# jinseikenai/glomeruli_segmentation

Measured on AMD Instinct MI355X. Metric: patches/sec (1024x512 RGB) ESPNet p=2 q=8 5 classes, HBM-resident, two batches in flight, higher is better.
Workload: dtype f32; 1 GPU; ESPNet p=2 q=8 encoder+decoder, batch=32 synthetic 1024x512 uint8 BGR tiles per GPU, normalise+forward+argmax+counts, inputs resident in HBM, steps rotate through 4 distinct batches, 2 batch(es) in flight (engine lanes, one HIP stream each) for `value`; global_batch=32, weights=espnet_fold1 (tests/golden), parallelism=tile-range per rank x1

## Files before the change

### glomeruli_segmentation_amd/_lib.py

```python
import ctypes
import os

_PKG = os.path.dirname(os.path.abspath(__file__))
LIB_PATH = os.path.join(_PKG, "libglomseg.so")
if os.environ.get("GLOMSEG_LIB") and os.environ.get("GLOMSEG_EXPERIMENT") == "1":
    LIB_PATH = os.environ["GLOMSEG_LIB"]

GS_OK = 0
GS_IN_U8_BGR_NHWC = 0
GS_IN_F32_NCHW = 1
ABI_VERSION = 10
GS_BUILD_DIAG = 1
GS_FORM_NONE = -1
GS_MAX_ENSEMBLE_C = 8
MAX_CROPS_PER_CALL = 64

STATUS_NAMES = {0: "GS_OK", 1: "GS_ERR_INVALID", 2: "GS_ERR_HIP", 3: "GS_ERR_NOMEM", 4: "GS_ERR_UNSUPPORTED",
                5: "GS_ERR_NODEVICE", 6: "GS_ERR_DEVICE_FAULT"}


class GlomsegError(RuntimeError):
    def __init__(self, status, message):
        super().__init__("%s: %s" % (STATUS_NAMES.get(status, status), message))
        self.status = status
# ... 95 lines not shown
    "gs_arc_length_closed": (ctypes.c_double, [_P, _I]),
    "gs_approx_poly_closed": (_I, [_P, _I, ctypes.c_double, _P]),
    "gs_wsi_paste_max": (_I, [_P, _I, _I, _I, _P, _I, _I, _I, _I, _P]),
    "gs_wsi_paste_max_lut": (_I, [_P, _I, _I, _I, _P, _P, _P, _I, _I, _I, _I, _P]),
    "gs_overlay_classmap": (_I, [_P, _P, _I, _I, _P, _I, ctypes.c_float, ctypes.c_float, _P, _P]),
    "gs_confusion_u8": (_I, [_P, _P, ctypes.c_longlong, _I, _P, _P]),
    "gs_wsi_eval_windows": (_I, [_I, _I, _I, _I, ctypes.POINTER(EvalSet), ctypes.POINTER(EvalSet), _P, _P, _I, _I, _P, _P, _P]),
    "gs_conv2d_nhwc": (_I, [_P, _I, _I, _I, _I, _P, _I, _I, _I, _P, _I, _I, _I, _P, _P]),
    "gs_conv2d_nhwc_form": (_I, [_I] * 10 + [ctypes.POINTER(ctypes.c_char_p)]),
    "gs_roialign": (_I, [_P, _I, _I, _I, _I, _P, _P, _I, _I, _P, _P]),
    "gs_nms": (_I, [_P, _P, _I, ctypes.c_float, ctypes.c_float, _I, _P, _P, _P]),
    "gs_detector_create": (_I, [_P, ctypes.POINTER(LayerDesc), _I, ctypes.POINTER(_P)]),
    "gs_detector_destroy": (None, [_P]),
    "gs_detector_max_detections": (_I, []),
    "gs_detector_num_proposals": (_I, []),
    "gs_detector_layer_info": (_I, [_I, ctypes.POINTER(ctypes.c_char_p)] + [ctypes.POINTER(_I)] * 6),
    "gs_detector_plan": (_I, [_I, _I, _I, ctypes.POINTER(DetectorPlan)]),
    "gs_detector_set_thresholds": (_I, [_P, ctypes.c_float, ctypes.c_float, ctypes.c_float]),
    "gs_detector_forward": (_I, [_P, _P, _I, _I, _I, _P, _P, _P, _P, _P, _P, _P, _P, _P]),
    "gs_detector_detect_host": (_I, [_P, ctypes.POINTER(_P), _I, _I, _I, _I, _P, _P, _P, _P]),
}

SCORING_PROTOTYPES = {
    "gs_espnet_score_crops": (_I, [_P, _P, ctypes.POINTER(CropDesc), _I, _I, _I, _I, _P, _P, _P]),
    "gs_espnet_segment_crops_host_scored": (_I, PROTOTYPES["gs_espnet_segment_crops_host"][1] + [ctypes.POINTER(CropScoring)]),
}

PLAN_PROTOTYPES = {
    "gs_espnet_plan_flags": (_I, [_I, _I, _I, _I, _I, _I, _I, _I, ctypes.POINTER(_I)]),
    "gs_espnet_pack_weights": (_I, [_P, ctypes.POINTER(LayerDesc), _I, _I, _I, _I, _I, _P, ctypes.c_size_t, ctypes.POINTER(ctypes.c_size_t),
                                ctypes.POINTER(WeightPiece), _I, ctypes.POINTER(_I)]),
    "gs_espnet_workspace_plan": (_I, [_I] * 7 + [ctypes.POINTER(ctypes.c_size_t)]),
}
GS_PLAN_LAZY_B2, GS_PLAN_L3C_IN_REDUCE, GS_PLAN_CLS_IN_L3 = 1, 2, 4

INSTANCE_PROTOTYPES = {
    "gs_instances_plan": (_I, [_I, _I, _I, _I, ctypes.POINTER(ctypes.c_size_t)]),
    "gs_slide_instances": (_I, [_P, _I, _I, _I, _I, _P, ctypes.c_size_t, _I, _P, _P, _P, _P, _P]),
}

_lib = None


def load():
    global _lib
    if _lib is not None:
        return _lib
    if not os.path.exists(LIB_PATH):
        raise ImportError(
            "%s is missing: build it with `python -m glomeruli_segmentation_amd.build` "
            "(hipcc --offload-arch=gfx950).  There is no CPU fallback." % LIB_PATH)
    lib = ctypes.CDLL(LIB_PATH, mode=ctypes.RTLD_GLOBAL)
    for name, (res, args) in list(PROTOTYPES.items()) + list(SCORING_PROTOTYPES.items()) + list(PLAN_PROTOTYPES.items()) + \
            list(INSTANCE_PROTOTYPES.items()):
        if name in PLAN_PROTOTYPES and not hasattr(lib, name):
            continue
        fn = getattr(lib, name)
        fn.restype = res
        fn.argtypes = args
    if lib.gs_abi_version() != ABI_VERSION:
        raise ImportError("libglomseg.so ABI %d != binding ABI %d: rebuild" % (lib.gs_abi_version(), ABI_VERSION))
    if (lib.gs_build_flags() & GS_BUILD_DIAG) and os.environ.get("GLOMSEG_ALLOW_DIAG") != "1":
        raise ImportError("%s is a -DGS_DIAG experiment build (its timing variants return wrong results by construction); "
                          "set GLOMSEG_ALLOW_DIAG=1 to load it for an A/B measurement" % LIB_PATH)
    _lib = lib
    return lib

# ... 10 lines not shown
```

### glomeruli_segmentation_amd/build.py

```python
import os
import subprocess
import sys
import tempfile

PKG = os.path.dirname(os.path.abspath(__file__))
CSRC = os.path.join(PKG, "csrc")
LIB = os.path.join(PKG, "libglomseg.so")
SOURCES = ["espnet.hip", "dec_tail.hip", "crops.hip", "detect_ops.hip", "detector.hip", "wsi_eval.hip", "instances.hip", "contours.cpp"]
HEADERS = ["gs_internal.h", "conv_mfma.h", "dec_tail.h", "dec_tail_args.h", "espnet_kernels.h", "espnet_facts.h", "espnet_weights.h", "workspace_plan.h", "crop_sample.h", "crop_plan.h", "instance_plan.h", "detect_math.h", "detect_plan.h", "host_copy.h", "host_jobs.h", "host_pipe.h",
           os.path.join("..", "..", "include", "glomseg.h"), os.path.join("..", "..", "include", "glomseg_scoring.h"),
           os.path.join("..", "..", "include", "glomseg_plan.h"), os.path.join("..", "..", "include", "glomseg_instances.h")]
FLAGS = ["-O3", "--offload-arch=gfx950", "-std=c++17", "-fPIC", "-Wall", "-Wno-unused-result",
         "-Wno-unused-value"]


def _sources():
    return [s for s in SOURCES if os.path.exists(os.path.join(CSRC, s))]


def _stale(lib):
    if not os.path.exists(lib):
        return True
    t = os.path.getmtime(lib)
    deps = [os.path.join(CSRC, s) for s in _sources() + HEADERS] + [os.path.abspath(__file__)]
    deps += [os.path.join(CSRC, f) for f in os.listdir(CSRC) if f.endswith(".h") or f.endswith(".inc")]
    return any(os.path.getmtime(d) > t for d in deps)


def build_lib(force=False, verbose=False, out=None, extra_flags=()):
    lib = os.path.abspath(out) if out else LIB
    if not (force or _stale(lib)):
        return lib
    hipcc = os.environ.get("HIPCC", "/opt/rocm/bin/hipcc")
    os.makedirs(os.path.dirname(lib), exist_ok=True)
    objdir = CSRC if out is None else tempfile.mkdtemp(prefix="glomseg_obj_")
    objs = []
    procs = []
    for s in _sources():
        o = os.path.join(objdir, s.replace(".hip", ".o").replace(".cpp", ".o"))
        objs.append(o)
        cmd = [hipcc] + FLAGS + list(extra_flags) + (["-x", "hip"] if s.endswith(".cpp") else []) + ["-c", os.path.join(CSRC, s), "-o", o]
        if verbose:
# ... 21 lines not shown
```

### glomeruli_segmentation_amd/csrc/espnet.hip

```cpp
#include <chrono>
#include <cmath>
#include <cstdio>
#include <cstdlib>
#include <functional>
#include <map>
#include <memory>
#include <string>
#include <thread>
#include <vector>

#include "../../include/glomseg_plan.h"
#include "conv_mfma.h"
#include "dec_tail_args.h"
#include "enc_head.h"
#include "enc_head_ens.h"
#include "espnet_config.h"
#include "forward_plan.h"
#include "espnet_kernels.h"
#include "espnet_weights.h"
#include "host_copy.h"
#include "host_pipe.h"
#include "workspace_plan.h"

namespace gs {

static thread_local std::string g_err;
void set_error(const char *fmt, ...)
{
    char buf[1024];
    va_list ap;
    va_start(ap, fmt);
    vsnprintf(buf, sizeof buf, fmt, ap);
    va_end(ap);
    g_err = buf;
}

#ifdef GS_DIAG
static bool getenv_flag(const char *name)
{
    const char *e = std::getenv(name);
    return e && std::atoi(e) != 0;
}
static bool no_vec() { return getenv_flag("GS_NO_VEC"); }
#else
static constexpr bool no_vec() { return false; }
#endif

enum KernelId {
    K_STEM, K_POOL, K_L2_C1S, K_L2_DOWN, K_L2_C1, K_L2_ESP, K_CAT_B2, K_L3_C1S, K_L3_DOWN, K_L3_C1, K_L3_ESP,
    K_DEC1, K_DEC2, K_DEC3, K_DEC_CONV, K_DEC4, K_DEC_TAIL, K_ENC_HEAD, K_ENC_HEAD_ENS, K_COUNT
};
static const char *kKernelNames[K_COUNT] = {
    "stem_kernel", "pool_kernel", "conv_l2_reduce_s2", "conv_l2_down_branches", "conv_l2_reduce_1x1",
    "conv_l2_esp_branches", "cat_b2_kernel", "conv_l3_reduce_s2", "conv_l3_down_branches", "conv_l3_reduce_1x1",
    "conv_l3_esp_branches", "dec1_kernel", "dec2_kernel", "dec3_kernel", "conv_dec_cbr", "dec4_kernel", "dec_tail_kernel",
    "enc_head_kernel", "enc_head_ens_kernel"};

struct Model : Workspace {
    int classes = 0, p = 0, q = 0;
    int cp = 0;
    bool encoder_only = false;
    int device = 0, num_cus = 256;
#ifdef GS_DIAG
    int variant = 0;
#else
    static constexpr int variant = 0;
#endif
    float *dblob = nullptr;
    EspnetOffsets w;

    void *ws = nullptr;
    size_t ws_bytes = 0;
    int ws_n = 0, ws_h = 0, ws_w = 0;
    float *prob = nullptr;
    size_t prob_bytes = 0;
    std::map<std::string, std::pair<Act, int>> stages;
    void set_stage(const std::string &name, const Act &act, int C)
    {
        for (auto it = stages.begin(); it != stages.end();)
            it = it->second.first.base == act.base ? stages.erase(it) : std::next(it);
        stages[name] = {act, C};
    }
    int last_n = 0;
    bool b2_lazy = false;

    bool profile = false;
    struct Ev { hipEvent_t a, b; int k; };
    std::vector<Ev> events;
    double prof_ms[K_COUNT] = {0};
    long long prof_launches[K_COUNT] = {0};
    double prof_flops[K_COUNT] = {0};
};

static gs_status layout_workspace(Model *m, int n, int H, int W)
{
    if (m->ws && n <= m->ws_n && H == m->ws_h && W == m->ws_w)
        return GS_OK;
    if (m->ws) {
        GS_HIP(hipDeviceSynchronize());
        GS_HIP(hipFree(m->ws));
        m->ws = nullptr;
    }
    WorkspacePlan plan;
    const gs_status st = plan_workspace(n, H, W, m->cp, m->p, m->encoder_only, plan);
    if (st != GS_OK)
        return st;
    void *ws = nullptr;
    if (hipMalloc(&ws, plan.bytes) != hipSuccess) {
        set_error("workspace allocation of %zu bytes failed (n=%d, %dx%d)", plan.bytes, n, H, W);
        return GS_ERR_NOMEM;
    }
    GS_HIP(hipMemset(ws, 0, plan.bytes));
    GS_HIP(hipDeviceSynchronize());
    static_cast<Workspace &>(*m) = plan.acts;
    int i = 0;
    for (Act *a : acts_of(*m))
        a->base = reinterpret_cast<float *>(static_cast<char *>(ws) + plan.at[i++]);
// ... 396 lines not shown
            }
            ca = with_cls(ca, 0);
        }
        return launch_l3_down(m, plan.l3_down, plan.cls_in_l3, m->w.l3_0.fused_next ? with_fused(ca, m->r3[rd3 ^ 1], 25) : ca, s);
    });
    bool have_r3 = m->w.l3_0.fused_next;
    m->set_stage("level3_reduce", m->r3[rd3], 25);
    rd3 ^= have_r3 ? 1 : 0;
    m->set_stage("level3_0", m->cc[0], 128);
    int cur3 = 0;
    for (int i = 0; i < m->q; ++i) {
        const int nxt = cur3 == 1 ? 2 : 1;
        const bool fuse_next = m->w.l3[i].fused_next;
        if (!have_r3)
            L.run(K_L3_C1, px3 * (128 * 25 * 2), [&] {
                return launch_l3_c1(m, conv_args(m->cc[cur3], wb + m->w.l3[i].c1, m->r3[rd3], nullptr, n), s);
            });
        L.run(K_L3_ESP, px3 * (25 * 9 * 128 * 2) + (fuse_next ? px3 * (128 * 25 * 2) : 0) + (i == m->q - 1 ? cls_flops : 0), [&] {
            const ConvArgs ca = conv_args(m->r3[rd3], wb + m->w.l3[i].br, m->cc[nxt], &m->cc[cur3], n);
            GS_DIAG_TRY(diag_l3_esp(m, ca, i, s, dst_));
            if (fuse_next)
                return launch_l3_esp_fused(m, plan.l3_esp_fused, with_fused(ca, m->r3[rd3 ^ 1], 25), i, s);
            const bool cls5 = plan.cls_in_l3 && i == m->q - 1;
            return launch_l3_esp_last(m, plan.l3_esp_last, cls5, cls5 ? with_cls(ca, 1) : ca, s);
        });
        have_r3 = fuse_next;
        rd3 ^= have_r3 ? 1 : 0;
        cur3 = nxt;
        m->set_stage("level3." + std::to_string(i), m->cc[cur3], 128);
    }
    return {cur3, lazy_b2};
}

template <int CLS>
static gs_status decode(Model *m, Launcher &L, const ForwardPlan &plan, const ForwardReq &r, const Encoded &enc)
{
    const float *wb = m->dblob;
    const hipStream_t s = r.s;
    const int n = r.n, H = r.H, W = r.W, H1 = H / 2, W1 = W / 2, H2 = H / 4, W2 = W / 4, H3 = H / 8, W3 = W / 8;
    const double px1 = (double)H1 * W1, px2 = (double)H2 * W2, px3 = (double)H3 * W3;
    const int ncls = m->classes;
    float *enc_logits = !m->encoder_only ? nullptr : r.logits ? r.logits : m->o2c.base;
    L.run(K_DEC1, (plan.cls_in_l3 ? 0 : px3 * (256 * ncls * 2)) + px3 * (ncls * ncls * 4 * 2), [&] {
        if constexpr (CLS == CLS_N) {
            if (plan.cls_in_l3) {
                Dec1SumsArgs a{};
                a.part = m->tt.base;
                a.psn = m->tt.sn;
                a.psc = H3 * W3;
                a.br = wb + m->w.br;
                a.wup = wb + m->w.wup3;
                a.out = view(m->o2c);
                a.N = n;
                a.H3 = H3;
                a.W3 = W3;
                a.classes = ncls;
                hipLaunchKernelGGL(dec1_sums_kernel<CLS>, dim3(blocks_for((long long)n * H3 * W3)), dim3(256), 0, s, a);
                return GS_OK;
            }
        }
        Dec1Args a{};
        a.c0 = view(m->cc[0]);
        a.clast = view(m->cc[enc.last]);
        a.b3w = wb + m->w.b3;
        a.br = m->encoder_only ? nullptr : wb + m->w.br;
        a.wup = m->encoder_only ? nullptr : wb + m->w.wup3;
        a.out = view(m->o2c);
        a.enc_logits = enc_logits;
        a.N = n;
        a.classes = ncls;
        constexpr int CB = CLS <= 5 ? 16 : CLS <= 8 ? 8 : 4;
        hipLaunchKernelGGL((dec1_kernel<CLS, CB>), dim3((unsigned)(((long long)n * H3 * W3 + 63) / 64)), dim3(256), 0, s, a);
        return GS_OK;
    });
    if (m->encoder_only) {
        if (r.mask)
            L.run(K_ENC_HEAD, (double)H * W * (ncls * 6), [&] {
                EncHeadArgs a{};
                a.logits = enc_logits;
                a.mask = r.mask;
                a.hist = r.hist;
                a.classes = ncls;
                a.H3 = H3;
                a.W3 = W3;
                launch_enc_head(a, n, s);
                return GS_OK;
            });
        return L.st;
    }
    m->set_stage("up_l3", m->o2c, ncls);

    L.run(K_DEC2, plan.l3c_in_reduce ? 0 : px2 * (131 * ncls * 2), [&] {
        Dec2Args a{};
        a.o2c = view(m->o2c);
        a.br = wb + m->w.cbr0;
        a.t = view(m->tt);
        a.N = n;
        a.classes = ncls;
        if constexpr (l3c_side_sums(CLS)) {
            if (plan.l3c_in_reduce) {
                a.a1 = view(m->l3c);
                hipLaunchKernelGGL(dec2_br_kernel<CLS>, dim3(blocks_for((long long)n * H2 * W2)), dim3(256), 0, s, a);
                return GS_OK;
            }
        }
        a.a1 = view(m->a1);
        a.raw = view(m->bb[0]);
        a.b2 = wb + m->w.b2;
        a.raw_c0 = 64;
        a.raw_cn = enc.lazy_b2 ? 64 : 0;
        a.w3c = wb + m->w.w3c;
        hipLaunchKernelGGL(dec2_kernel<CLS>, dim3((unsigned)(((long long)n * H2 * W2 + 63) / 64)), dim3(256), 0, s, a);
        return GS_OK;
    });
    if (ncls == CLS)
        m->set_stage("combine_t", m->tt, 2 * CLS);
    if constexpr (dec3_on_mfma(CLS)) {
        L.run(K_DEC3, px2 * (2 * ncls * 9 * ncls * 2), [&] {
            return launch_dec3<CLS>(m, plan.dec3, conv_args(m->tt, wb + m->w.wcc_mfma, m->t3, nullptr, n), s);
        });
        L.run(K_DEC3, px2 * (ncls * ncls * 4 * 2), [&] {
            Dec3Args a{};
            a.t = view(m->t3);
            a.wup = wb + m->w.wup2;
            a.bnu = wb + m->w.bnu2;
            a.e = view(m->ee);
            a.N = n;
            a.classes = ncls;
            hipLaunchKernelGGL(dec3b_kernel<CLS>, dim3(blocks_for((long long)n * H2 * W2)), dim3(256), 0, s, a);
            return GS_OK;
        });
    } else {
        L.run(K_DEC3, px2 * (2 * ncls * 9 * ncls * 2) + px2 * (ncls * ncls * 4 * 2), [&] {
            Dec3Args a{};
            a.t = view(m->tt);
            a.wc = wb + m->w.wcc;
            a.bnc = wb + m->w.bncc;
            a.wup = wb + m->w.wup2;
            a.bnu = wb + m->w.bnu2;
            a.e = view(m->ee);
            a.N = n;
            a.classes = ncls;
            hipLaunchKernelGGL(dec3_kernel<CLS>, dim3(blocks_for((long long)n * H2 * W2)), dim3(256), 0, s, a);
            return GS_OK;
        });
    }
    m->set_stage("up_l2", m->ee, ncls);
    if constexpr (dec_tail_fused(CLS)) {
        L.run(K_DEC_TAIL, px1 * ((19 + CLS) * 9 * CLS * 2) + px1 * (CLS * CLS * 4 * 2), [&] {
            DecTailArgs a{};
            a.in = m->a0c.base;
            a.in_sn = m->a0c.sn;
            a.in_sc = m->a0c.sc;
            a.in_pitch = m->a0c.pitch;
            a.in_off = m->a0c.off;
            a.in_img_bytes = (unsigned)(m->a0c.sn * sizeof(float));
            a.wpack = wb + m->w.wtail;
            a.logits = r.logits;
            a.mask = r.mask;
            a.hist = ens_finishes((int)r.role) ? r.hist : nullptr;
            a.prob = r.prob;
            a.ens_mode = (int)r.role;
            a.ens_w = r.ens_w;
            if (r.logits) {
// ... 365 lines not shown
    GS_REQUIRE(h && in, "gs_espnet_forward: null handle or input");
    GS_REQUIRE(lane >= 0 && lane <= (int)h->lanes.size(), "lane %d does not exist (gs_espnet_set_lanes)", lane);
    gs_status st = check_shape(n, height, width);
    if (st != GS_OK) return st;
    GS_REQUIRE(in_format == GS_IN_U8_BGR_NHWC || in_format == GS_IN_F32_NCHW, "unknown input format %d", in_format);
    GS_REQUIRE(in_format != GS_IN_U8_BGR_NHWC || (mean && std), "uint8 input needs mean and std");
    GS_REQUIRE(logits || mask, "nothing to compute: logits and mask are both NULL");
    GS_REQUIRE(!hist || mask, "hist requires the mask output");
    if (in_format == GS_IN_U8_BGR_NHWC)
        for (int i = 0; i < 3; ++i)
            GS_REQUIRE(std[i] != 0.0f, "std[%d] is zero", i);
    ForwardReq r;
    r.in = in, r.in_format = in_format, r.n = n, r.H = height, r.W = width;
    r.mean = mean, r.stdv = std, r.logits = logits, r.mask = mask, r.hist = hist, r.s = static_cast<hipStream_t>(hip_stream);
    return espnet_forward(h, lane, r);
}

gs_status gs_espnet_read_stage(gs_espnet *h, const char *stage, int image, float *dst, size_t cap, int dims[3])
{
    GS_REQUIRE(h && stage && dims, "gs_espnet_read_stage: null argument");
    Model &m = h->m;
    auto it = m.stages.find(stage);
    GS_REQUIRE(it != m.stages.end(), "stage '%s' was not produced by the last forward", stage);
    GS_REQUIRE(image >= 0 && image < m.last_n, "image index %d out of range", image);
    const Act &a = it->second.first;
    const int C = it->second.second;
    dims[0] = C;
    dims[1] = a.H;
    dims[2] = a.W;
    const size_t count = (size_t)C * a.H * a.W;
    if (!dst)
        return GS_OK;
    GS_REQUIRE(cap >= count, "destination too small for stage '%s'", stage);
    float *tmp = nullptr;
    GS_HIP(hipMalloc(reinterpret_cast<void **>(&tmp), count * sizeof(float)));
    hipLaunchKernelGGL(unpad_kernel, dim3(blocks_for((long long)count)), dim3(256), 0, 0, view(a), image, C, tmp);
    if (m.b2_lazy && std::string(stage) == "b2")
        hipLaunchKernelGGL(b2_apply_kernel, dim3(blocks_for((long long)64 * a.H * a.W)), dim3(256), 0, 0, tmp, m.dblob + m.w.b2, a.H * a.W, 64, 64);
    hipError_t e = hipMemcpy(dst, tmp, count * sizeof(float), hipMemcpyDeviceToHost);
    hipFree(tmp);
    GS_HIP(e);
    return GS_OK;
}

gs_status gs_espnet_block_forward(gs_espnet *h, int kind, int level, int index, const float *in, int height, int width,
                                  float *out)
{
    GS_REQUIRE(h && in && out, "gs_espnet_block_forward: null argument");
    GS_REQUIRE((kind == 0 || kind == 1) && (level == 2 || level == 3), "kind must be 0/1 and level 2/3");
    GS_REQUIRE(height >= 1 && width >= 1, "empty input");
    Model &m = h->m;
    GS_REQUIRE(kind == 1 || (index >= 0 && index < (level == 2 ? m.p : m.q)), "no ESP block %d at level %d", index, level);
    GS_REQUIRE(kind == 0 || (height % 2 == 0 && width % 2 == 0), "the down-sampler needs an even input size");
    const int up = kind == 0 ? (level == 2 ? 4 : 8) : (level == 2 ? 2 : 4);
    gs_status st = layout_workspace(&m, 1, height * up, width * up);
    if (st != GS_OK) return st;
    const float *wb = m.dblob;
    const Act &src = kind == 0 ? (level == 2 ? m.bb[0] : m.cc[0]) : (level == 2 ? m.a0 : m.a1);
    const Act &dst = level == 2 ? (kind == 0 ? m.bb[1] : m.bb[0]) : (kind == 0 ? m.cc[1] : m.cc[0]);
    const Act &red = level == 2 ? m.r2[0] : m.r3[0];
    const int cin = kind == 0 ? (level == 2 ? 64 : 128) : (level == 2 ? 19 : 131);
    const int cout = level == 2 ? 64 : 128;
    GS_REQUIRE(src.H == height && src.W == width, "internal: workspace level size mismatch");
    const size_t nin = (size_t)cin * height * width, nout = (size_t)cout * dst.H * dst.W;
    float *tmp = nullptr;
    GS_HIP(hipMalloc(reinterpret_cast<void **>(&tmp), (nin > nout ? nin : nout) * sizeof(float)));
// ... 25 lines not shown
    };
    rc = body();
    hipFree(tmp);
    m.stages.clear();
    return rc;
}

gs_status gs_espnet_plan_forward(int n, int height, int width, int p, int q, int classes, int num_cus, int *out_forms, int cap,
                                 int *n_out)
{
    GS_REQUIRE(n_out, "gs_espnet_plan_forward: null argument");
    gs_status st = check_shape(n, height, width);
    if (st != GS_OK) return st;
    GS_REQUIRE(p >= 0 && q >= 0 && num_cus > 0, "gs_espnet_plan_forward: p and q must be non-negative, num_cus positive");
    if (classes < 2 || classes > 20) {
        set_error("gs_espnet_plan_forward: classes must be 2..20 (got %d)", classes);
        return GS_ERR_UNSUPPORTED;
    }
    *n_out = kLaunchClassCount;
    if (!out_forms)
        return GS_OK;
    GS_REQUIRE(cap >= kLaunchClassCount, "gs_espnet_plan_forward: %d entries needed, room for %d", kLaunchClassCount, cap);
    plan_forward(n, height, width, p, q, padded_classes(classes), num_cus, no_vec()).codes(out_forms);
    return GS_OK;
}

gs_status gs_espnet_plan_flags(int n, int height, int width, int p, int q, int classes, int encoder_only, int num_cus, int *flags)
{
    GS_REQUIRE(flags, "gs_espnet_plan_flags: null argument");
    int count = 0;
    gs_status st = gs_espnet_plan_forward(n, height, width, p, q, classes, num_cus, nullptr, 0, &count);
    if (st != GS_OK) return st;
    const ForwardPlan pl = plan_forward(n, height, width, p, q, padded_classes(classes), num_cus, no_vec(), encoder_only != 0);
    *flags = (pl.lazy_b2 ? GS_PLAN_LAZY_B2 : 0) | (pl.l3c_in_reduce ? GS_PLAN_L3C_IN_REDUCE : 0) | (pl.cls_in_l3 ? GS_PLAN_CLS_IN_L3 : 0);
    return GS_OK;
}

gs_status gs_espnet_form_info(int launch_class, int form, const char **name, int *pixels_per_lane)
{
    GS_REQUIRE(launch_class >= 0 && launch_class < kLaunchClassCount, "no launch class %d", launch_class);
    const LaunchClassInfo &c = kLaunchClasses[launch_class];
    GS_REQUIRE(form >= GS_FORM_NONE && form < c.n_forms, "launch class %s has no form %d", c.name, form);
    if (name) *name = form == GS_FORM_NONE ? c.name : c.forms[form].name;
    if (pixels_per_lane) *pixels_per_lane = form == GS_FORM_NONE ? 0 : c.forms[form].pixels_per_lane;
    return GS_OK;
}

gs_status gs_espnet_profile_enable(gs_espnet *h, int on)
{
    GS_REQUIRE(h, "null handle");
    h->m.profile = on != 0;
    return GS_OK;
}

gs_status gs_espnet_profile_read(gs_espnet *h, gs_kernel_time *out, int cap, int *n_out)
{
    GS_REQUIRE(h && n_out, "null argument");
    Model &m = h->m;
    for (auto &ev : m.events) {
        GS_HIP(hipEventSynchronize(ev.b));
        float ms = 0.0f;
        GS_HIP(hipEventElapsedTime(&ms, ev.a, ev.b));
        m.prof_ms[ev.k] += ms;
        m.prof_launches[ev.k] += 1;
        hipEventDestroy(ev.a);
        hipEventDestroy(ev.b);
    }
// ... 111 lines not shown
```

### glomeruli_segmentation_amd/csrc/espnet_facts.h

```cpp
#pragma once
#include <cstddef>

#include "../../include/glomseg.h"

namespace gs {

void set_error(const char *fmt, ...);

static inline long long round_up(long long a, long long b) { return (a + b - 1) / b * b; }

struct Act {
    float *base = nullptr;
    long long sn = 0;
    int sc = 0;
    int pitch = 0;
    int off = 0;
    int C = 0, Cp = 0;
    int H = 0, W = 0;
    size_t bytes(int n) const { return (size_t)n * sn * sizeof(float); }
};

constexpr int SIDE_REC = 8;
constexpr int SIDE_ZROWS = 16;
constexpr int side_table_floats(int CINP) { return (CINP + SIDE_ZROWS) * SIDE_REC; }
// ... 4 lines not shown
};
constexpr ConvImage conv_image(int CINP, int TAPS, int NDIL, int NOUT1, int NOUT, bool bn, bool dual = false, int fuse_nacc = 0)
{
    ConvImage im{};
    im.nrow = NOUT1 > NOUT ? NOUT1 : NOUT;
    im.cout = NOUT1 + (NDIL - 1) * NOUT;
    im.w = NDIL * TAPS * CINP * im.nrow;
    im.bn = (bn ? 3 * im.cout : 0) + (dual ? 3 * im.cout : 0);
    im.tab = NDIL * fuse_nacc * 64;
    im.total = (im.w + im.bn + im.tab + 3) / 4 * 4;
    return im;
}
constexpr int conv_wfloats(int CINP, int TAPS, int NDIL, int NOUT1, int NOUT, bool bn, bool dual = false, int fuse_nacc = 0)
{
    return conv_image(CINP, TAPS, NDIL, NOUT1, NOUT, bn, dual, fuse_nacc).total;
}

#ifndef CFG_FUSE_L3
#define CFG_FUSE_L3 2
#endif
#ifndef CFG_FUSE_L2
#define CFG_FUSE_L2 1
#endif

constexpr int padded_classes(int classes) { return classes == 5 ? 5 : (classes + 3) / 4 * 4; }
constexpr bool b2_is_lazy(int p) { return p > 0; }
constexpr bool l2_c1_fused(int i, int p) { return CFG_FUSE_L2 && i < p; }
constexpr bool l3_c1_fused(int i, int q) { return (CFG_FUSE_L3 == 2 || (CFG_FUSE_L3 == 1 && i == 0)) && i < q; }
constexpr bool dec3_on_mfma(int cp) { return cp >= 12; }
constexpr bool l3c_side_sums(int cp) { return cp == 5; }
constexpr bool cls_side_sums(int cp, int q) { return cp == 5 && q >= 1 && l3_c1_fused(0, q); }
constexpr int CLS_PART_PLANES = 20;
constexpr bool dec_tail_fused(int cp) { return cp == 5; }

constexpr int DT_A_FLOATS = 18 * 64;
constexpr int DT_PACK_FLOATS = DT_A_FLOATS + 16 + 100;

}
```

### glomeruli_segmentation_amd/csrc/forward_plan.h

```cpp
#pragma once
#include "espnet_config.h"

namespace gs {

constexpr int cfg_pixels(int, int, int, int, int, int, int, int, int p, int) { return p; }

constexpr int dec_mt(int cp) { return cp <= 16 ? 16 : 32; }
constexpr int dec_pixels(int cp) { return cp <= 16 ? 8 : 4; }

#define GS_FORMS_L2_DOWN(X)                              \
    X(P2S_VEC, "CFG_L2_BR_P2S+F_VEC", cfg_pixels(CFG_L2_BR_P2S))                                  \
    X(P4S_VEC_SKIP, "CFG_L2_BR_P4S+F_VEC+F_SKIP_PAD", cfg_pixels(CFG_L2_BR_P4S))                  \
    X(P4_VEC, "CFG_L2_BR_P4+F_VEC", cfg_pixels(CFG_L2_BR_P4))                                     \
    X(P4, "CFG_L2_BR_P4", 0)                                                                      \
    X(UNFUSED_P4_VEC, "unfused CFG_L2_BR_P4+F_VEC", cfg_pixels(CFG_L2_BR_P4))                     \
    X(UNFUSED_P4, "unfused CFG_L2_BR_P4", 0)
#define GS_FORMS_L2_ESP_FUSED(X)                        \
    X(P2S_VEC, "CFG_L2_BR_P2S+F_VEC", cfg_pixels(CFG_L2_BR_P2S))                                  \
    X(P4_VEC, "CFG_L2_BR_P4+F_VEC", cfg_pixels(CFG_L2_BR_P4))                                     \
    X(P4, "CFG_L2_BR_P4", 0)                                                                      \
    X(UNFUSED_P4_VEC, "unfused CFG_L2_BR_P4+F_VEC", cfg_pixels(CFG_L2_BR_P4))                     \
    X(UNFUSED_P4, "unfused CFG_L2_BR_P4", 0)
#define GS_FORMS_L2_ESP_LAST(X)             \
    X(P2S_VEC, "CFG_L2_BR_P2S+F_VEC", cfg_pixels(CFG_L2_BR_P2S))                                  \
// ... 46 lines not shown
    C(dec_conv, GS_FORMS_DEC_CONV)

struct FormInfo {
    const char *name;
    int pixels_per_lane;
};
struct LaunchClassInfo {
    const char *name;
    const FormInfo *forms;
    int n_forms;
};

#define GS_FORM_ID(id, name, ppl) id,
#define GS_FORM_INFO(id, name, ppl) {name, ppl},
#define GS_CLASS_ENUM(cls, FORMS) enum class cls : int { none = -1, FORMS(GS_FORM_ID) };
#define GS_CLASS_FORMS(cls, FORMS)                                          \
    constexpr FormInfo kForms_##cls[] = {FORMS(GS_FORM_INFO)};              \
    constexpr int pixels_per_lane(form::cls f) { return kForms_##cls[(int)f].pixels_per_lane; }
#define GS_CLASS_INFO(cls, FORMS) {#cls, kForms_##cls, (int)(sizeof kForms_##cls / sizeof kForms_##cls[0])},
#define GS_PLAN_MEMBER(cls, FORMS) form::cls cls = form::cls::none;
#define GS_PLAN_CODE(cls, FORMS) *out++ = (int)cls;
namespace form {
GS_LAUNCH_CLASSES(GS_CLASS_ENUM)
}
GS_LAUNCH_CLASSES(GS_CLASS_FORMS)
constexpr LaunchClassInfo kLaunchClasses[] = {GS_LAUNCH_CLASSES(GS_CLASS_INFO)};
constexpr int kLaunchClassCount = (int)(sizeof kLaunchClasses / sizeof kLaunchClasses[0]);

struct ForwardPlan {
    GS_LAUNCH_CLASSES(GS_PLAN_MEMBER)
    bool lazy_b2 = false;
    bool l3c_in_reduce = false;
    bool cls_in_l3 = false;
    void codes(int *out) const { GS_LAUNCH_CLASSES(GS_PLAN_CODE) }
};
#undef GS_FORM_ID
#undef GS_FORM_INFO
#undef GS_CLASS_ENUM
#undef GS_CLASS_FORMS
#undef GS_CLASS_INFO
#undef GS_PLAN_MEMBER
#undef GS_PLAN_CODE

template <typename F>
constexpr bool vec_fits(F v, int w, bool no_vec)
{
    return !no_vec && w % pixels_per_lane(v) == 0;
}

constexpr form::l2_down unfused_l2_down(int W2, bool no_vec)
{
    return vec_fits(form::l2_down::UNFUSED_P4_VEC, W2, no_vec) ? form::l2_down::UNFUSED_P4_VEC : form::l2_down::UNFUSED_P4;
}
constexpr form::l2_esp_fused unfused_l2_esp(int W2, bool no_vec)
{
    return vec_fits(form::l2_esp_fused::UNFUSED_P4_VEC, W2, no_vec) ? form::l2_esp_fused::UNFUSED_P4_VEC : form::l2_esp_fused::UNFUSED_P4;
}
constexpr form::l3_down unfused_l3_down(int W3, bool no_vec)
{
    return vec_fits(form::l3_down::UNFUSED_BR_VEC, W3, no_vec) ? form::l3_down::UNFUSED_BR_VEC : form::l3_down::UNFUSED_BR;
}
constexpr form::l3_esp_last whole_row_l3_esp(int W3, bool no_vec)
{
    return vec_fits(form::l3_esp_last::BR_VEC, W3, no_vec) ? form::l3_esp_last::BR_VEC : form::l3_esp_last::P2;
}

inline ForwardPlan plan_forward(int n, int H, int W, int p, int q, int cp, int num_cus, bool no_vec, bool encoder_only = false)
{
    namespace f = form;
    const int W1 = W / 2, H2 = H / 4, W2 = W / 4, H3 = H / 8, W3 = W / 8;
    const long long cus = num_cus;
    ForwardPlan pl;
    pl.lazy_b2 = b2_is_lazy(p);
    pl.l3c_in_reduce = !encoder_only && l3c_side_sums(cp);
    pl.cls_in_l3 = !encoder_only && cls_side_sums(cp, q);

    const bool small2 = CFG_SMALL2_WAVES > 0 && (long long)n * H2 * cdiv(W2, 64) * 2 <= cus * CFG_SMALL2_WAVES &&
                        vec_fits(f::l2_down::P2S_VEC, W2, no_vec);
    if (!l2_c1_fused(0, p))
        pl.l2_down = unfused_l2_down(W2, no_vec);
    else if (small2)
        pl.l2_down = f::l2_down::P2S_VEC;
    else if (CFG_L2_DOWN_SKIP && vec_fits(f::l2_down::P4S_VEC_SKIP, W2, no_vec))
        pl.l2_down = f::l2_down::P4S_VEC_SKIP;
    else
        pl.l2_down = vec_fits(f::l2_down::P4_VEC, W2, no_vec) ? f::l2_down::P4_VEC : f::l2_down::P4;
    if (p > 1) {
        if (!l2_c1_fused(1, p))
            pl.l2_esp_fused = unfused_l2_esp(W2, no_vec);
        else if (small2)
            pl.l2_esp_fused = f::l2_esp_fused::P2S_VEC;
        else
            pl.l2_esp_fused = vec_fits(f::l2_esp_fused::P4_VEC, W2, no_vec) ? f::l2_esp_fused::P4_VEC : f::l2_esp_fused::P4;
    }
    if (p > 0)
        pl.l2_esp_last = small2                                            ? f::l2_esp_last::P2S_VEC
                         : vec_fits(f::l2_esp_last::P4_VEC, W2, no_vec) ? f::l2_esp_last::P4_VEC
                                                                          : f::l2_esp_last::P4;
    if (!pl.lazy_b2)
        pl.cat_b2 = f::cat_b2::KERNEL;

    if (!pl.lazy_b2)
        pl.l3_reduce = f::l3_reduce::C1S;
    else
        pl.l3_reduce = (long long)n * H3 * cdiv(W3, 128) * 4 <= cus * 8 ? f::l3_reduce::BNL_P1 : f::l3_reduce::BNL;
    const bool small3 = (long long)n * H3 * cdiv(W3, 64) * 2 <= cus * CFG_SMALL3_WAVES && !no_vec;
    if (!l3_c1_fused(0, q))
        pl.l3_down = unfused_l3_down(W3, no_vec);
// ... 36 lines not shown
```

### glomeruli_segmentation_amd/engine.py

```python
import ctypes
import functools

import numpy as np
import torch

from . import _lib


def _to_numpy(v):
    if isinstance(v, torch.Tensor):
        return v.detach().cpu().numpy()
    return np.asarray(v)


def pack_state_dict(state_dict):
    items = []
    total = 0
    for name, v in state_dict.items():
        a = _to_numpy(v)
        if a.dtype.kind != "f":
            continue
        a = np.ascontiguousarray(a, dtype=np.float32)
        if a.ndim > 4:
            raise ValueError("tensor %s has %d dims" % (name, a.ndim))
# ... 230 lines not shown


@functools.lru_cache(maxsize=None)
def forward_forms():
    lib = _lib.load()
    table = []
    name, ppl = ctypes.c_char_p(), ctypes.c_int()
    while lib.gs_espnet_form_info(len(table), _lib.GS_FORM_NONE, ctypes.byref(name), ctypes.byref(ppl)) == _lib.GS_OK:
        k, cls, forms = len(table), name.value.decode(), []
        while lib.gs_espnet_form_info(k, len(forms), ctypes.byref(name), ctypes.byref(ppl)) == _lib.GS_OK:
            forms.append((name.value.decode(), ppl.value))
        table.append((cls, tuple(forms)))
    return tuple(table)


def plan_forward(n, height, width, p, q, classes, num_cus):
    lib = _lib.load()
    table = forward_forms()
    codes, count = (ctypes.c_int * len(table))(), ctypes.c_int()
    _lib.check(lib.gs_espnet_plan_forward(n, height, width, p, q, classes, num_cus, codes, len(table), ctypes.byref(count)))
    return {cls: forms[codes[k]][0] for k, (cls, forms) in enumerate(table) if codes[k] != _lib.GS_FORM_NONE}


def plan_flags(n, height, width, p, q, classes, num_cus, encoder_only=False):
    flags = ctypes.c_int()
    _lib.check(_lib.load().gs_espnet_plan_flags(n, height, width, p, q, classes, int(bool(encoder_only)), num_cus, ctypes.byref(flags)))
    return {"lazy_b2": bool(flags.value & _lib.GS_PLAN_LAZY_B2), "l3c_in_reduce": bool(flags.value & _lib.GS_PLAN_L3C_IN_REDUCE)}


def plan_cls_in_l3(n, height, width, p, q, classes, num_cus, encoder_only=False):
    flags = ctypes.c_int()
    _lib.check(_lib.load().gs_espnet_plan_flags(n, height, width, p, q, classes, int(bool(encoder_only)), num_cus, ctypes.byref(flags)))
    return bool(flags.value & _lib.GS_PLAN_CLS_IN_L3)


def pack_weights(state_dict, classes=5, p=2, q=8, encoder_only=False):
    lib = _lib.load()
    src, table = pack_state_dict(state_dict)
    head = (src.ctypes.data_as(ctypes.c_void_p), table, len(table), classes, p, q, int(bool(encoder_only)))
    n, n_pieces = ctypes.c_size_t(), ctypes.c_int()
    _lib.check(lib.gs_espnet_pack_weights(*head, None, 0, ctypes.byref(n), None, 0, ctypes.byref(n_pieces)))
    blob, pieces = np.empty(n.value, dtype=np.float32), (_lib.WeightPiece * n_pieces.value)()
    _lib.check(lib.gs_espnet_pack_weights(*head, blob.ctypes.data_as(ctypes.c_void_p), blob.size, ctypes.byref(n), pieces, len(pieces),
                                          ctypes.byref(n_pieces)))
    return blob, {pc.name.decode(): (pc.offset, pc.floats) for pc in pieces}


def workspace_bytes(n, height, width, p, q, classes, encoder_only=False):
    b = ctypes.c_size_t()
    _lib.check(_lib.load().gs_espnet_workspace_plan(n, height, width, p, q, classes, int(bool(encoder_only)), ctypes.byref(b)))
    return b.value


def crop_preprocess(crop_u8, mean, std, out_h, out_w, out=None):
    lib = _lib.load()
    crop_u8 = crop_u8.contiguous()
    h, w, _ = crop_u8.shape
    if out is None:
        out = torch.empty((3, out_h, out_w), dtype=torch.float32, device=crop_u8.device)
    with torch.cuda.device(crop_u8.device):
        _lib.check(lib.gs_crop_preprocess(crop_u8.data_ptr(), h, w, _lib.fptr3(mean), _lib.fptr3(std), out_h, out_w,
                                          out.data_ptr(), _stream_ptr(crop_u8.device)))
    return out


def mask_resize_nearest(mask, out_h, out_w):
# ... 170 lines not shown
```

### include/glomseg_plan.h

```cpp
#ifndef GLOMSEG_PLAN_H
#define GLOMSEG_PLAN_H

#include "glomseg.h"

#ifdef __cplusplus
extern "C" {
#endif

#define GS_PLAN_LAZY_B2 1
#define GS_PLAN_L3C_IN_REDUCE 2
enum { GS_PLAN_CLS_IN_L3 = 4 };

gs_status gs_espnet_plan_flags(int n, int height, int width, int p, int q, int classes, int encoder_only, int num_cus, int *flags);


typedef struct gs_weight_piece {
    char name[32];
    long long offset, floats;
} gs_weight_piece;

gs_status gs_espnet_pack_weights(const float *blob, const gs_layer_desc *table, int n_layers, int classes, int p, int q,
                                 int encoder_only, float *out, size_t cap, size_t *n_floats, gs_weight_piece *pieces, int piece_cap,
                                 int *n_pieces);

gs_status gs_espnet_workspace_plan(int n, int height, int width, int p, int q, int classes, int encoder_only, size_t *bytes);

#ifdef __cplusplus
}
#endif

#endif
```

Baseline: 11810 patches/s.

## Fuse decoder dec1 sums, dec2 BR and dec3 conv/upsample into one tiled kernel

Adds a dec_mid kernel for five-class networks that computes the level-3 class sums, the 2x transposed upsample, the BN-PReLU of the concatenation, the 3x3 conv and the final 2x upsample in one pass. Intermediates are kept in a shared-memory tile with a halo, so the separate dec1 and dec2 launches and their o2c/tt round-trips to HBM are no longer needed. Stage dumps of up_l3/combine_t lazily recompute the skipped buffers. The cost is recomputation of halo pixels and a serial loop over ten input channels per thread.

Measured after the change: 11750 patches/s. No clear change (-0.5%).

```diff
diff --git a/glomeruli_segmentation_amd/_lib.py b/glomeruli_segmentation_amd/_lib.py
--- a/glomeruli_segmentation_amd/_lib.py
+++ b/glomeruli_segmentation_amd/_lib.py
@@ -151,7 +151,7 @@
                                 ctypes.POINTER(WeightPiece), _I, ctypes.POINTER(_I)]),
     "gs_espnet_workspace_plan": (_I, [_I] * 7 + [ctypes.POINTER(ctypes.c_size_t)]),
 }
-GS_PLAN_LAZY_B2, GS_PLAN_L3C_IN_REDUCE, GS_PLAN_CLS_IN_L3 = 1, 2, 4
+GS_PLAN_LAZY_B2, GS_PLAN_L3C_IN_REDUCE, GS_PLAN_CLS_IN_L3, GS_PLAN_DEC_MID_FUSED = 1, 2, 4, 8
 
 INSTANCE_PROTOTYPES = {
     "gs_instances_plan": (_I, [_I, _I, _I, _I, ctypes.POINTER(ctypes.c_size_t)]),
diff --git a/glomeruli_segmentation_amd/build.py b/glomeruli_segmentation_amd/build.py
--- a/glomeruli_segmentation_amd/build.py
+++ b/glomeruli_segmentation_amd/build.py
@@ -7,7 +7,7 @@
 CSRC = os.path.join(PKG, "csrc")
 LIB = os.path.join(PKG, "libglomseg.so")
 SOURCES = ["espnet.hip", "dec_tail.hip", "crops.hip", "detect_ops.hip", "detector.hip", "wsi_eval.hip", "instances.hip", "contours.cpp"]
-HEADERS = ["gs_internal.h", "conv_mfma.h", "dec_tail.h", "dec_tail_args.h", "espnet_kernels.h", "espnet_facts.h", "espnet_weights.h", "workspace_plan.h", "crop_sample.h", "crop_plan.h", "instance_plan.h", "detect_math.h", "detect_plan.h", "host_copy.h", "host_jobs.h", "host_pipe.h",
+HEADERS = ["gs_internal.h", "conv_mfma.h", "dec_tail.h", "dec_tail_args.h", "espnet_kernels.h", "dec_mid.h", "espnet_facts.h", "espnet_weights.h", "workspace_plan.h", "crop_sample.h", "crop_plan.h", "instance_plan.h", "detect_math.h", "detect_plan.h", "host_copy.h", "host_jobs.h", "host_pipe.h",
            os.path.join("..", "..", "include", "glomseg.h"), os.path.join("..", "..", "include", "glomseg_scoring.h"),
            os.path.join("..", "..", "include", "glomseg_plan.h"), os.path.join("..", "..", "include", "glomseg_instances.h")]
 FLAGS = ["-O3", "--offload-arch=gfx950", "-std=c++17", "-fPIC", "-Wall", "-Wno-unused-result",
diff --git a/glomeruli_segmentation_amd/csrc/dec_mid.h b/glomeruli_segmentation_amd/csrc/dec_mid.h
--- /dev/null
+++ b/glomeruli_segmentation_amd/csrc/dec_mid.h
@@ -0,0 +1,157 @@
+#pragma once
+#include "espnet_kernels.h"
+
+namespace gs {
+
+struct DecMidArgs {
+    const float *part;
+    long long psn;
+    int psc;
+    const float *br;
+    const float *wup3;
+    ActV l3c;
+    const float *cbr0;
+    const float *wc;
+    const float *bnc;
+    const float *wup2;
+    const float *bnu;
+    ActV e;
+    int N, H3, W3;
+    int classes;
+};
+
+__device__ __forceinline__ f32x2_t fma2(float w, f32x2_t v, f32x2_t acc)
+{
+    return __builtin_elementwise_fma(f32x2_t{w, w}, v, acc);
+}
+__device__ __forceinline__ f32x2_t bn_prelu2(f32x2_t v, const float *bnp, int C, int c)
+{
+    const f32x2_t t = v * bnp[c] + bnp[C + c];
+    const float alpha = bnp[2 * C + c], pin = alpha <= 1.0f ? __builtin_inff() : -__builtin_inff();
+    const f32x2_t u = alpha * t;
+    return f32x2_t{__builtin_amdgcn_fmed3f(t.x, u.x, pin), __builtin_amdgcn_fmed3f(t.y, u.y, pin)};
+}
+
+static inline unsigned dec_mid_blocks(int n, int H3, int W3)
+{
+    return (unsigned)((long long)n * ((2 * H3 + DEC_MID_TY - 1) / DEC_MID_TY) * ((2 * W3 + DEC_MID_TX - 1) / DEC_MID_TX));
+}
+
+template <int CLS>
+__global__ void __launch_bounds__(256) dec_mid_kernel(const DecMidArgs a)
+{
+    static_assert(CLS == 5, "the fused middle exists for the five-class networks (cls_side_sums, l3c_side_sums)");
+    constexpr int TY = DEC_MID_TY, TX = DEC_MID_TX, LY = TY + 2, LX = TX + 2;
+    constexpr int PY = TY / 2 + 2, PX = TX / 2 + 2;
+    constexpr int RP = 256 / TX, NP = TY / RP;
+    static_assert(TY % 2 == 0 && TX % 2 == 0 && 256 % TX == 0 && TY % RP == 0 && PY * PX <= 256, "tile shape");
+    __shared__ float tile[2 * CLS][LY][LX];
+    const int H2 = 2 * a.H3, W2 = 2 * a.W3;
+    const int tiles_x = (W2 + TX - 1) / TX, tiles_y = (H2 + TY - 1) / TY;
+    const int x0 = (int)(blockIdx.x % tiles_x) * TX;
+    const int y0 = (int)(blockIdx.x / tiles_x % tiles_y) * TY;
+    const int n = (int)(blockIdx.x / ((unsigned)tiles_x * tiles_y));
+    const int ncls = real_classes<CLS>(a.classes);
+
+    if (threadIdx.x < PY * PX) {
+        const int iy = threadIdx.x / PX, ix = threadIdx.x % PX;
+        const int y = y0 / 2 - 1 + iy, x = x0 / 2 - 1 + ix;
+        const bool in = (unsigned)y < (unsigned)a.H3 && (unsigned)x < (unsigned)a.W3;
+        float s[CLS], c3[CLS][2][2];
+#pragma unroll
+        for (int k = 0; k < CLS; ++k) {
+            s[k] = 0.0f;
+#pragma unroll
+            for (int dy = 0; dy < 2; ++dy)
+                c3[k][dy][0] = c3[k][dy][1] = 0.0f;
+        }
+        if (in) {
+            const float *pp = a.part + (long long)n * a.psn + y * a.W3 + x;
+            float g[4][CLS];
+#pragma unroll
+            for (int j = 0; j < 4; ++j)
+#pragma unroll
+                for (int k = 0; k < CLS; ++k)
+                    g[j][k] = pp[(long long)(j * CLS + k) * a.psc];
+#pragma unroll
+            for (int k = 0; k < CLS; ++k)
+#pragma unroll
+                for (int dy = 0; dy < 2; ++dy) {
+                    const float2 v = *reinterpret_cast<const float2 *>(at(a.l3c, n, k, 2 * y + dy, 2 * x));
+                    c3[k][dy][0] = v.x;
+                    c3[k][dy][1] = v.y;
+                }
+#pragma unroll
+            for (int k = 0; k < CLS; ++k) {
+                s[k] = (g[0][k] + g[1][k]) + (g[2][k] + g[3][k]);
+                s[k] = s[k] * a.br[k] + a.br[CLS + k];
+            }
+            zero_padding_lanes<CLS>(s, ncls);
+        }
+#pragma unroll
+        for (int o = 0; o < CLS; ++o)
+#pragma unroll
+            for (int dy = 0; dy < 2; ++dy)
+#pragma unroll
+                for (int dx = 0; dx < 2; ++dx) {
+                    float t = 0.0f;
+#pragma unroll
+                    for (int i = 0; i < CLS; ++i)
+                        t = fmaf(s[i], a.wup3[((i * CLS + o) * 2 + dy) * 2 + dx], t);
+                    const float v0 = bn_prelu(c3[o][dy][dx], a.cbr0, 2 * CLS, o);
+                    const float v1 = bn_prelu(t, a.cbr0, 2 * CLS, CLS + o);
+                    const int ly = 2 * iy + dy - 1, lx = 2 * ix + dx - 1;
+                    if ((unsigned)ly < (unsigned)LY && (unsigned)lx < (unsigned)LX) {
+                        tile[o][ly][lx] = in ? v0 : 0.0f;
+                        tile[CLS + o][ly][lx] = in ? v1 : 0.0f;
+                    }
+                }
+    }
+    __syncthreads();
+
+    static_assert(NP == 2, "two pixels per thread: the packed chains");
+    const int lx = threadIdx.x % TX, ly = threadIdx.x / TX;
+    f32x2_t s[CLS];
+#pragma unroll
+    for (int k = 0; k < CLS; ++k)
+        s[k] = f32x2_t{0.0f, 0.0f};
+#pragma unroll 1
+    for (int c = 0; c < 2 * CLS; ++c) {
+#pragma unroll
+        for (int ky = 0; ky < 3; ++ky)
+#pragma unroll
+            for (int kx = 0; kx < 3; ++kx) {
+                const f32x2_t v = {tile[c][ly + ky][lx + kx], tile[c][ly + RP + ky][lx + kx]};
+#pragma unroll
+                for (int k = 0; k < CLS; ++k)
+                    s[k] = fma2(a.wc[((k * 2 * CLS + c) * 3 + ky) * 3 + kx], v, s[k]);
+            }
+    }
+#pragma unroll
+    for (int k = 0; k < CLS; ++k)
+        s[k] = bn_prelu2(s[k], a.bnc, CLS, k);
+    const int x = x0 + lx;
+    const bool ok[NP] = {x < W2 && y0 + ly < H2, x < W2 && y0 + ly + RP < H2};
+#pragma unroll
+    for (int o = 0; o < CLS; ++o) {
+        f32x2_t up[2][2];
+#pragma unroll
+        for (int dy = 0; dy < 2; ++dy)
+#pragma unroll
+            for (int dx = 0; dx < 2; ++dx) {
+                f32x2_t t = {0.0f, 0.0f};
+#pragma unroll
+                for (int i = 0; i < CLS; ++i)
+                    t = fma2(a.wup2[((i * CLS + o) * 2 + dy) * 2 + dx], s[i], t);
+                up[dy][dx] = bn_prelu2(t, a.bnu, CLS, o);
+            }
+#pragma unroll
+        for (int j = 0; j < NP; ++j)
+#pragma unroll
+            for (int dy = 0; dy < 2; ++dy)
+                if (ok[j] && o < ncls)
+                    *reinterpret_cast<float2 *>(at(a.e, n, o, 2 * (y0 + ly + j * RP) + dy, 2 * x)) = make_float2(up[dy][0][j], up[dy][1][j]);
+    }
+}
+
+}
diff --git a/glomeruli_segmentation_amd/csrc/espnet.hip b/glomeruli_segmentation_amd/csrc/espnet.hip
--- a/glomeruli_segmentation_amd/csrc/espnet.hip
+++ b/glomeruli_segmentation_amd/csrc/espnet.hip
@@ -17,6 +17,7 @@
 #include "espnet_config.h"
 #include "forward_plan.h"
 #include "espnet_kernels.h"
+#include "dec_mid.h"
 #include "espnet_weights.h"
 #include "host_copy.h"
 #include "host_pipe.h"
@@ -83,6 +84,7 @@
     }
     int last_n = 0;
     bool b2_lazy = false;
+    bool mid_lazy = false;
 
     bool profile = false;
     struct Ev { hipEvent_t a, b; int k; };
@@ -545,6 +547,34 @@
     return {cur3, lazy_b2};
 }
 
+static void launch_dec1_sums(const Model *m, int n, hipStream_t s)
+{
+    const int H3 = m->o2c.H / 2, W3 = m->o2c.W / 2;
+    Dec1SumsArgs a{};
+    a.part = m->tt.base;
+    a.psn = m->tt.sn;
+    a.psc = H3 * W3;
+    a.br = m->dblob + m->w.br;
+    a.wup = m->dblob + m->w.wup3;
+    a.out = view(m->o2c);
+    a.N = n;
+    a.H3 = H3;
+    a.W3 = W3;
+    a.classes = m->classes;
+    hipLaunchKernelGGL(dec1_sums_kernel<CLS_N>, dim3(blocks_for((long long)n * H3 * W3)), dim3(256), 0, s, a);
+}
+static void launch_dec2_br(const Model *m, int n, hipStream_t s)
+{
+    Dec2Args a{};
+    a.a1 = view(m->l3c);
+    a.o2c = view(m->o2c);
+    a.br = m->dblob + m->w.cbr0;
+    a.t = view(m->tt);
+    a.N = n;
+    a.classes = m->classes;
+    hipLaunchKernelGGL(dec2_br_kernel<CLS_N>, dim3(blocks_for((long long)n * m->tt.H * m->tt.W)), dim3(256), 0, s, a);
+}
+
 template <int CLS>
 static gs_status decode(Model *m, Launcher &L, const ForwardPlan &plan, const ForwardReq &r, const Encoded &enc)
 {
@@ -554,38 +584,30 @@
     const double px1 = (double)H1 * W1, px2 = (double)H2 * W2, px3 = (double)H3 * W3;
     const int ncls = m->classes;
     float *enc_logits = !m->encoder_only ? nullptr : r.logits ? r.logits : m->o2c.base;
-    L.run(K_DEC1, (plan.cls_in_l3 ? 0 : px3 * (256 * ncls * 2)) + px3 * (ncls * ncls * 4 * 2), [&] {
-        if constexpr (CLS == CLS_N) {
-            if (plan.cls_in_l3) {
-                Dec1SumsArgs a{};
-                a.part = m->tt.base;
-                a.psn = m->tt.sn;
-                a.psc = H3 * W3;
-                a.br = wb + m->w.br;
-                a.wup = wb + m->w.wup3;
-                a.out = view(m->o2c);
-                a.N = n;
-                a.H3 = H3;
-                a.W3 = W3;
-                a.classes = ncls;
-                hipLaunchKernelGGL(dec1_sums_kernel<CLS>, dim3(blocks_for((long long)n * H3 * W3)), dim3(256), 0, s, a);
-                return GS_OK;
+    const bool mid_fused = CLS == CLS_N && plan.dec_mid_fused;
+    m->mid_lazy = mid_fused;
+    if (!mid_fused)
+        L.run(K_DEC1, (plan.cls_in_l3 ? 0 : px3 * (256 * ncls * 2)) + px3 * (ncls * ncls * 4 * 2), [&] {
+            if constexpr (CLS == CLS_N) {
+                if (plan.cls_in_l3) {
+                    launch_dec1_sums(m, n, s);
+                    return GS_OK;
+                }
             }
-        }
-        Dec1Args a{};
-        a.c0 = view(m->cc[0]);
-        a.clast = view(m->cc[enc.last]);
-        a.b3w = wb + m->w.b3;
-        a.br = m->encoder_only ? nullptr : wb + m->w.br;
-        a.wup = m->encoder_only ? nullptr : wb + m->w.wup3;
-        a.out = view(m->o2c);
-        a.enc_logits = enc_logits;
-        a.N = n;
-        a.classes = ncls;
-        constexpr int CB = CLS <= 5 ? 16 : CLS <= 8 ? 8 : 4;
-        hipLaunchKernelGGL((dec1_kernel<CLS, CB>), dim3((unsigned)(((long long)n * H3 * W3 + 63) / 64)), dim3(256), 0, s, a);
-        return GS_OK;
-    });
+            Dec1Args a{};
+            a.c0 = view(m->cc[0]);
+            a.clast = view(m->cc[enc.last]);
+            a.b3w = wb + m->w.b3;
+            a.br = m->encoder_only ? nullptr : wb + m->w.br;
+            a.wup = m->encoder_only ? nullptr : wb + m->w.wup3;
+            a.out = view(m->o2c);
+            a.enc_logits = enc_logits;
+            a.N = n;
+            a.classes = ncls;
+            constexpr int CB = CLS <= 5 ? 16 : CLS <= 8 ? 8 : 4;
+            hipLaunchKernelGGL((dec1_kernel<CLS, CB>), dim3((unsigned)(((long long)n * H3 * W3 + 63) / 64)), dim3(256), 0, s, a);
+            return GS_OK;
+        });
     if (m->encoder_only) {
         if (r.mask)
             L.run(K_ENC_HEAD, (double)H * W * (ncls * 6), [&] {
@@ -603,29 +625,29 @@
     }
     m->set_stage("up_l3", m->o2c, ncls);
 
-    L.run(K_DEC2, plan.l3c_in_reduce ? 0 : px2 * (131 * ncls * 2), [&] {
-        Dec2Args a{};
-        a.o2c = view(m->o2c);
-        a.br = wb + m->w.cbr0;
-        a.t = view(m->tt);
-        a.N = n;
-        a.classes = ncls;
-        if constexpr (l3c_side_sums(CLS)) {
-            if (plan.l3c_in_reduce) {
-                a.a1 = view(m->l3c);
-                hipLaunchKernelGGL(dec2_br_kernel<CLS>, dim3(blocks_for((long long)n * H2 * W2)), dim3(256), 0, s, a);
-                return GS_OK;
+    if (!mid_fused)
+        L.run(K_DEC2, plan.l3c_in_reduce ? 0 : px2 * (131 * ncls * 2), [&] {
+            if constexpr (l3c_side_sums(CLS)) {
+                if (plan.l3c_in_reduce) {
+                    launch_dec2_br(m, n, s);
+                    return GS_OK;
+                }
             }
-        }
-        a.a1 = view(m->a1);
-        a.raw = view(m->bb[0]);
-        a.b2 = wb + m->w.b2;
-        a.raw_c0 = 64;
-        a.raw_cn = enc.lazy_b2 ? 64 : 0;
-        a.w3c = wb + m->w.w3c;
-        hipLaunchKernelGGL(dec2_kernel<CLS>, dim3((unsigned)(((long long)n * H2 * W2 + 63) / 64)), dim3(256), 0, s, a);
-        return GS_OK;
-    });
+            Dec2Args a{};
+            a.o2c = view(m->o2c);
+            a.br = wb + m->w.cbr0;
+            a.t = view(m->tt);
+            a.N = n;
+            a.classes = ncls;
+            a.a1 = view(m->a1);
+            a.raw = view(m->bb[0]);
+            a.b2 = wb + m->w.b2;
+            a.raw_c0 = 64;
+            a.raw_cn = enc.lazy_b2 ? 64 : 0;
+            a.w3c = wb + m->w.w3c;
+            hipLaunchKernelGGL(dec2_kernel<CLS>, dim3((unsigned)(((long long)n * H2 * W2 + 63) / 64)), dim3(256), 0, s, a);
+            return GS_OK;
+        });
     if (ncls == CLS)
         m->set_stage("combine_t", m->tt, 2 * CLS);
     if constexpr (dec3_on_mfma(CLS)) {
@@ -643,6 +665,29 @@
             hipLaunchKernelGGL(dec3b_kernel<CLS>, dim3(blocks_for((long long)n * H2 * W2)), dim3(256), 0, s, a);
             return GS_OK;
         });
+    } else if (mid_fused) {
+        if constexpr (CLS == CLS_N)
+            L.run(K_DEC3, px3 * (ncls * ncls * 4 * 2) + px2 * (2 * ncls * 9 * ncls * 2) + px2 * (ncls * ncls * 4 * 2), [&] {
+                DecMidArgs a{};
+                a.part = m->tt.base;
+                a.psn = m->tt.sn;
+                a.psc = H3 * W3;
+                a.br = wb + m->w.br;
+                a.wup3 = wb + m->w.wup3;
+                a.l3c = view(m->l3c);
+                a.cbr0 = wb + m->w.cbr0;
+                a.wc = wb + m->w.wcc;
+                a.bnc = wb + m->w.bncc;
+                a.wup2 = wb + m->w.wup2;
+                a.bnu = wb + m->w.bnu2;
+                a.e = view(m->ee);
+                a.N = n;
+                a.H3 = H3;
+                a.W3 = W3;
+                a.classes = ncls;
+                hipLaunchKernelGGL(dec_mid_kernel<CLS>, dim3(dec_mid_blocks(n, H3, W3)), dim3(256), 0, s, a);
+                return GS_OK;
+            });
     } else {
         L.run(K_DEC3, px2 * (2 * ncls * 9 * ncls * 2) + px2 * (ncls * ncls * 4 * 2), [&] {
             Dec3Args a{};
@@ -1074,6 +1119,12 @@
     if (!dst)
         return GS_OK;
     GS_REQUIRE(cap >= count, "destination too small for stage '%s'", stage);
+    if (m.mid_lazy && (std::string(stage) == "up_l3" || std::string(stage) == "combine_t")) {
+        launch_dec1_sums(&m, m.last_n, 0);
+        launch_dec2_br(&m, m.last_n, 0);
+        GS_HIP(hipGetLastError());
+        m.mid_lazy = false;
+    }
     float *tmp = nullptr;
     GS_HIP(hipMalloc(reinterpret_cast<void **>(&tmp), count * sizeof(float)));
     hipLaunchKernelGGL(unpad_kernel, dim3(blocks_for((long long)count)), dim3(256), 0, 0, view(a), image, C, tmp);
@@ -1165,7 +1216,8 @@
     gs_status st = gs_espnet_plan_forward(n, height, width, p, q, classes, num_cus, nullptr, 0, &count);
     if (st != GS_OK) return st;
     const ForwardPlan pl = plan_forward(n, height, width, p, q, padded_classes(classes), num_cus, no_vec(), encoder_only != 0);
-    *flags = (pl.lazy_b2 ? GS_PLAN_LAZY_B2 : 0) | (pl.l3c_in_reduce ? GS_PLAN_L3C_IN_REDUCE : 0) | (pl.cls_in_l3 ? GS_PLAN_CLS_IN_L3 : 0);
+    *flags = (pl.lazy_b2 ? GS_PLAN_LAZY_B2 : 0) | (pl.l3c_in_reduce ? GS_PLAN_L3C_IN_REDUCE : 0) | (pl.cls_in_l3 ? GS_PLAN_CLS_IN_L3 : 0) |
+             (pl.dec_mid_fused ? GS_PLAN_DEC_MID_FUSED : 0);
     return GS_OK;
 }
 
diff --git a/glomeruli_segmentation_amd/csrc/espnet_facts.h b/glomeruli_segmentation_amd/csrc/espnet_facts.h
--- a/glomeruli_segmentation_amd/csrc/espnet_facts.h
+++ b/glomeruli_segmentation_amd/csrc/espnet_facts.h
@@ -60,6 +60,8 @@
 constexpr bool cls_side_sums(int cp, int q) { return cp == 5 && q >= 1 && l3_c1_fused(0, q); }
 constexpr int CLS_PART_PLANES = 20;
 constexpr bool dec_tail_fused(int cp) { return cp == 5; }
+constexpr int DEC_MID_TY = 16;
+constexpr int DEC_MID_TX = 32;
 
 constexpr int DT_A_FLOATS = 18 * 64;
 constexpr int DT_PACK_FLOATS = DT_A_FLOATS + 16 + 100;
diff --git a/glomeruli_segmentation_amd/csrc/forward_plan.h b/glomeruli_segmentation_amd/csrc/forward_plan.h
--- a/glomeruli_segmentation_amd/csrc/forward_plan.h
+++ b/glomeruli_segmentation_amd/csrc/forward_plan.h
@@ -102,6 +102,7 @@
     bool lazy_b2 = false;
     bool l3c_in_reduce = false;
     bool cls_in_l3 = false;
+    bool dec_mid_fused = false;
     void codes(int *out) const { GS_LAUNCH_CLASSES(GS_PLAN_CODE) }
 };
 #undef GS_FORM_ID
@@ -144,6 +145,7 @@
     pl.lazy_b2 = b2_is_lazy(p);
     pl.l3c_in_reduce = !encoder_only && l3c_side_sums(cp);
     pl.cls_in_l3 = !encoder_only && cls_side_sums(cp, q);
+    pl.dec_mid_fused = pl.cls_in_l3 && pl.l3c_in_reduce;
 
     const bool small2 = CFG_SMALL2_WAVES > 0 && (long long)n * H2 * cdiv(W2, 64) * 2 <= cus * CFG_SMALL2_WAVES &&
                         vec_fits(f::l2_down::P2S_VEC, W2, no_vec);
diff --git a/glomeruli_segmentation_amd/engine.py b/glomeruli_segmentation_amd/engine.py
--- a/glomeruli_segmentation_amd/engine.py
+++ b/glomeruli_segmentation_amd/engine.py
@@ -286,6 +286,12 @@
     flags = ctypes.c_int()
     _lib.check(_lib.load().gs_espnet_plan_flags(n, height, width, p, q, classes, int(bool(encoder_only)), num_cus, ctypes.byref(flags)))
     return bool(flags.value & _lib.GS_PLAN_CLS_IN_L3)
+
+
+def plan_dec_mid_fused(n, height, width, p, q, classes, num_cus, encoder_only=False):
+    flags = ctypes.c_int()
+    _lib.check(_lib.load().gs_espnet_plan_flags(n, height, width, p, q, classes, int(bool(encoder_only)), num_cus, ctypes.byref(flags)))
+    return bool(flags.value & _lib.GS_PLAN_DEC_MID_FUSED)
 
 
 def pack_weights(state_dict, classes=5, p=2, q=8, encoder_only=False):
diff --git a/include/glomseg_plan.h b/include/glomseg_plan.h
--- a/include/glomseg_plan.h
+++ b/include/glomseg_plan.h
@@ -10,6 +10,7 @@
 #define GS_PLAN_LAZY_B2 1
 #define GS_PLAN_L3C_IN_REDUCE 2
 enum { GS_PLAN_CLS_IN_L3 = 4 };
+enum { GS_PLAN_DEC_MID_FUSED = 8 };
 
 gs_status gs_espnet_plan_flags(int n, int height, int width, int p, int q, int classes, int encoder_only, int num_cus, int *flags);
 
```
